# meharkhurana03/cm3d

Hardware: AMD Instinct MI355X
Metric: pseudo-label frames/sec on nuScenes-shaped sweeps (higher is better)
Workload: dtype f32; 1 GPU; c2: 256 frames/GPU x (35000x1 pts, 6 cams, 20 masks 1600x900), masks resident as rle; frames_per_gpu=256, points_per_frame=35000, masks_per_frame=20, lane_points=50000, mask_input=rle, batches_in_flight=4, distinct_batches=4, cloud_materialised=False

## Files before the change

cm3d_amd/_lib.py:

```python
import ctypes as C
import os

_HERE = os.path.dirname(os.path.abspath(__file__))
LIB_PATH = os.environ.get("CM3D_LIB") or os.path.join(_HERE, "libcm3d_hip.so")

ABI_VERSION = 5
CAM_STRIDE = 64
SWEEP_XF_STRIDE = 24
MAX_CAMS = 8
MAX_MASKS_PER_FRAME = 1024
BOX_STRIDE = 10
MEDOID_TILE = 64
STATUS_WORDS = 4
BBOX_STRIDE = 8
MAX_MATCH_BOXES = 1024
MAX_FUSED_SWEEPS = 16
MATCH_BOX_STRIDE = 6
OBB_ROT_STRIDE = 9
WM_BOX_STRIDE = 8
WM_BREAKDOWNS = 16
WM_CUTOFFS = 101
WM_SWEEP_MAX_ALPHAS = 1024
RAW_QUADS = 3

_p, _i32, _i64, _f32 = C.c_void_p, C.c_int32, C.c_int64, C.c_float

SIGNATURES = {
    "cm3d_abi_version": (_i32, []),
    "cm3d_project_workgroups_per_cu": (_i32, [_i32]),
    "cm3d_error_string": (C.c_char_p, [_i32]),
    "cm3d_removed_words": (_i64, [_i32, _i32]),
    "cm3d_batch_begin": (_i32, [_p, _p, _i32, _p, _i64, _p]),
    "cm3d_sweep_prep": (_i32, [_p, _i32, _p, _p, _i32, _i32, _p, _p, _i32, _f32, _p, _i32, _p, _p, _p, _p]),
    "cm3d_rle_workspace_bytes": (_i64, [_i32]),
    "cm3d_rle_to_dense": (_i32, [_p, _p, _i32, _i32, _i32, _i32, _p, _p, _i64, _p]),
    "cm3d_erode_pack": (_i32, [_p, _i32, _i32, _i32, _p, _p, _p]),
    "cm3d_rle_erode_pack": (_i32, [_p, _p, _i32, _i32, _i32, _i32, _p, _p, _p, _i64, _p]),
    "cm3d_rle_erode_pack_begin": (_i32, [_p, _p, _i32, _i32, _i32, _i32, _p, _p, _p, _i64, _p, _p, _i32, _p, _i64, _p]),
    "cm3d_rle_erode_pack_sized": (_i32, [_p, _p, _i32, _i32, _i32, _i32, _p, _p, _p, _p, _i64, _p]),
    "cm3d_rle_erode_pack_sized_begin": (_i32, [_p, _p, _i32, _i32, _i32, _i32, _p, _p, _p, _p, _i64, _p, _p, _i32, _p, _i64, _p]),
    "cm3d_project_workspace_bytes": (_i64, [_i32, _i32, _i32]),
    "cm3d_project_hit_rows": (_i32, [_p, _i64, _i32, _i32, _i32, _p, _p]),
    "cm3d_project_culling": (_i32, [_p, _i64, _i32, _i32, _i32, _p, _p]),
    "cm3d_project_hits": (_i32, [_p, _p, _i32, _i32, _i32, _p, _i32, _p, _p, _p, _p, _i32, _i32, _i32, _f32, _i32,
                                 _p, _p, _p, _p, _i64, _p, _p, _p]),
    "cm3d_sweep_project_hits": (_i32, [_p, _i32, _p, _p, _i32, _i32, _p, _p, _f32, _p, _i32, _p, _p, _i32, _i32, _i32, _p, _i32, _p, _p,
                                       _p, _p, _i32, _i32, _i32, _f32, _i32, _p, _p, _p, _p, _i64, _p, _p, _p]),
    "cm3d_compact_hits": (_i32, [_p, _i32, _i32, _i32, _i32, _p, _i32, _p, _p, _p, _i32, _p, _p, _p, _p, _p, _p, _p, _p, _i32, _p, _p, _p,
                                 _i64, _p]),
    "cm3d_tile_work_bytes": (_i64, [_i32, _i32]),
    "cm3d_selftest_sqrt": (_i32, [C.c_uint32, C.c_uint32, _p, _p, _p]),
    "cm3d_selftest_div": (_i32, [C.c_uint64, C.c_uint64, _p, _p]),
    "cm3d_selftest_mfma": (_i32, [C.c_uint64, _i32, _p, _p]),
    "cm3d_medoid_workspace_bytes": (_i64, [_i32, _i32]),
    "cm3d_medoid": (_i32, [_p, _p, _p, _i32, _p, _p, _p, _i32, _p, _p, _p, _p, _p, _i64, _p]),
    "cm3d_medoid2": (_i32, [_p, _p, _p, _i32, _p, _p, _p, _i32, _p, _p, _p, _p, _p, _i64, _i32, _p, _p]),
    "cm3d_lane_grid_bytes": (_i64, [_i32, _i32]),
    "cm3d_lane_grid_build": (_i32, [_p, _p, _i32, _i32, _p, _i64, _p]),
    "cm3d_lane_nn_workspace_bytes": (_i64, [_i32]),
    "cm3d_lane_nn": (_i32, [_p, _p, _p, _i32, _p, _p, _p, _i32, _i32, _p, _p, _p, _p, _i64, _p]),
    "cm3d_circle_nms": (_i32, [_p, _p, _p, _p, _p, _i32, _p, _i32, _p, _p]),
    "cm3d_box_nms": (_i32, [_p, _p, _p, _i32, _i32, _p, _p, _p, _p, _p, _p, _p, _p, _p, _p, _p, _i32, _p, _p, _p, _p, _p]),
    "cm3d_centroid_transform": (_i32, [_p, _p, _p, _i32, _p, _p, _p]),
    "cm3d_bev_match_workspace_bytes": (_i64, [_i64]),
    "cm3d_bev_match": (_i32, [_p, _p, _i32, _p, _p, _i32, _p, _i32, _i64, C.c_double, _p, _p, _p, _p, _p, _i64, _p]),
    "cm3d_obb_workspace_bytes": (_i64, [_i32, _i32]),
    "cm3d_obb": (_i32, [_p, _p, _i32, _i32, _p, _p, _p, _p, _p, _i64, _p]),
    "cm3d_selftest_obb_yaw": (_i32, [_p, _i32, _p, _p]),
    "cm3d_waymo_metrics_workspace_bytes": (_i64, [_i64]),
    "cm3d_waymo_metrics": (_i32, [_p, _p, _p, _p, _p, _p, _p, _p, _p, _p, _i32, _i64, _i32, _p, _p, _p, _p, _i64, _p]),
    "cm3d_waymo_metrics_sweep_workspace_bytes": (_i64, [_i64]),
    "cm3d_waymo_metrics_sweep": (_i32, [_p, _p, _p, _p, _p, _p, _p, _p, _p, _p, _p, _p, _p, _i32, _i64, _p, _i32, _p, _p, _p, _p, _i64, _p]),
    "cm3d_lift_pass": (_i32, [_p, _p]),
    "cm3d_pipe_exec_streams_for": (_i32, [_i32, _i32]),
    "cm3d_pipe_create": (_p, [_i32, _i32, _p]),
    "cm3d_pipe_destroy": (None, [_p]),
    "cm3d_pipe_exec_streams": (_i32, [_p]),
    "cm3d_pipe_submit": (_i32, [_p, _i32, _p]),
    "cm3d_pipe_submit_timed": (_i32, [_p, _i32, _p, _p, _p]),
    "cm3d_pipe_acquire": (_i32, [_p, _i32]),
    "cm3d_pipe_release": (_i32, [_p, _i32]),
    "cm3d_pipe_wait": (_i32, [_p, _i32]),
    "cm3d_pipe_pin": (_i32, [_p]),
    "cm3d_pipe_last_stream": (_i32, [_p, _i32]),
}


class LiftPassDesc(C.Structure):
    _fields_ = (
        [("size", _i64)]
        + [(n, _p) for n in ("rle_counts", "rle_off", "packed", "bbox", "rle_ws")] + [("rle_ws_bytes", _i64)]
        + [(n, _p) for n in ("status", "hit_count", "removed_bits")] + [("removed_words", _i64)]
        + [(n, _p) for n in ("raw", "intensity", "sweep_row_off", "sweep_xf", "frame_sweep_off", "points", "pt_off", "cams", "mask_off",
                             "mask_cam", "hit_words", "pg_ws")] + [("pg_ws_bytes", _i64)]
        + [(n, _p) for n in ("hit_off", "tile_off", "hit_idx", "hit_xyz", "tile_work", "medoid_pos", "centroid", "colsum", "ws")]
        + [("ws_bytes", _i64), ("md_feedback", _p)]
        + [(n, _p) for n in ("centroid_g", "mask_frame", "lane", "lane_off", "frame_lane", "grid", "lane_idx", "lane_dist", "class_id", "score",
                             "prior_wlh", "is_vehicle", "nms_group", "nms_thr", "ego_xyz", "box", "flags")]
        + [(n, _i32) for n in ("n_masks", "total_runs", "W", "H", "raw_stride", "n_sweeps", "max_sweeps_per_frame", "pt_cap", "n_frames",
                               "max_pts_per_frame", "n_cams", "planes", "idx_cap", "n_tables", "n_lane_points", "n_classes", "md_hint")]
        + [("halfw", _f32), ("min_dist", _f32)])


class Cm3dError(RuntimeError):
    pass


_lib = None


def lib():
    global _lib
    if _lib is None:
        if not os.path.exists(LIB_PATH):
            raise Cm3dError(
                f"{LIB_PATH} is missing: build it with `python -c 'import __graft_entry__ as g; g.build()'` "
                "(hipcc --offload-arch=gfx950).  There is no CPU fallback for the lifting path.")
        handle = C.CDLL(LIB_PATH)
        for name, (res, args) in SIGNATURES.items():
            fn = getattr(handle, name)
            fn.restype = res
            fn.argtypes = args
        if handle.cm3d_abi_version() != ABI_VERSION:
            raise Cm3dError("libcm3d_hip.so ABI version mismatch")
        _lib = handle
    return _lib


def check(code, what):
    if code != 0:
        msg = lib().cm3d_error_string(code).decode()
        raise Cm3dError(f"{what}: {msg} ({code})")
```

cm3d_amd/csrc/boxes.hip:

```cpp
#include "common.h"

#define LG_MAX_CELLS 32768
#define LG_CELL0 4.0f
#define LG_MAX_RINGS 64
#define LG_BIG_CELL 12
#define LG_BUILD_THREADS 1024

struct LaneGrid { float x0, y0, h, inv_h; int gw, gh, cell_base; float margin; };
struct LanePt { float x, y; int idx, pad; };

static __device__ __forceinline__ int lg_cell_coord(float v, float v0, float inv_h, int n)
{
    int c = (int)floorf((v - v0) * inv_h);
    return c < 0 ? 0 : (c >= n ? n - 1 : c);
}

__global__ __launch_bounds__(LG_BUILD_THREADS) void k_lane_grid_build(const float *__restrict__ lane,
                                                                      const int32_t *__restrict__ lane_off,
                                                                      LaneGrid *__restrict__ grids, int32_t *__restrict__ cell_start,
                                                                      LanePt *__restrict__ sorted)
{
    extern __shared__ __align__(16) int s_cell[];
    __shared__ float s_red[4][16];
    __shared__ int s_part[16];
// ... 137 lines not shown
                const int sg = s0 + lane;
                int row, c0, c1;
                if (r_lo == 0) { row = qj - 2 + sg; c0 = qi - 2; c1 = qi + 2; }
                else if (sg < w) { row = qj - r_hi + sg; c0 = qi - r_hi; c1 = qi + r_hi; }
                else if (sg < 2 * w) { row = qj + r_lo + (sg - w); c0 = qi - r_hi; c1 = qi + r_hi; }
                else {
                    const int m = sg - 2 * w;
                    row = qj - r_lo + 1 + (m >> 1);
                    if (m & 1) { c0 = qi + r_lo; c1 = qi + r_hi; } else { c0 = qi - r_hi; c1 = qi - r_lo; }
                }
                c0 = max(c0, 0); c1 = min(c1, g.gw - 1);
                const bool seg_ok = sg < nseg && row >= 0 && row < g.gh && c0 <= c1;
                const int rowc = min(max(row, 0), g.gh - 1), c0c = min(c0, g.gw - 1), c1c = max(c1, 0);
                int a = cs[rowc * g.gw + c0c], b = cs[rowc * g.gw + c1c + 1];
                if (!seg_ok) { a = 0; b = 0; }
                visit(a, b);
            }
            r_done = r_hi;
            const double wb = cm3d_wave_reduce_t(sbest, [](double a, double b) { return fmin(a, b); });
            if (wb < (double)r_done * (double)g.h - (double)g.margin) { resolved = true; break; }
            if (qi - r_done <= 0 && qi + r_done >= g.gw - 1 && qj - r_done <= 0 && qj + r_done >= g.gh - 1) { resolved = true; break; }
        }
    }
    if (!resolved) {
        const int32_t *cs = cell_start + g.cell_base;
        const int a = cs[0], b = cs[g.gw * g.gh];
        for (int q0 = a; q0 < b; q0 += 8 * 64) {
            LanePt p[8];
#pragma unroll
            for (int v = 0; v < 8; ++v) {
                const int q = q0 + v * 64 + lane;
                p[v] = q < b ? sorted[q] : LanePt{0.f, 0.f, 0, 0};
            }
#pragma unroll
            for (int v = 0; v < 8; ++v) {
                if (q0 + v * 64 + lane >= b) continue;
                const double dx = cx - (double)p[v].x, dy = cy - (double)p[v].y;
                lg_consider(dx * dx + dy * dy, p[v].idx, d2cut, sbest, jbest);
            }
        }
    }
    {
        const Cm3dDistIdx best = cm3d_wave_argmin(sbest, jbest);
        sbest = best.s; jbest = best.j;
    }
    if (lane == 0) {
        if (jbest == 0x7FFFFFFF) jbest = 0;
        lane_idx[k] = jbest;
        lane_dist[k] = sbest;
    }
}

static inline size_t lg_align(size_t v) { return (v + 255) & ~(size_t)255; }

struct LgLayout { LaneGrid *grids; int32_t *cell_start; LanePt *sorted; };
static inline LgLayout lg_layout(void *grid, int n_tables, int n_lane_points)
{
    char *w = (char *)grid;
    LgLayout l;
    l.grids = (LaneGrid *)w;          w += lg_align(sizeof(LaneGrid) * (size_t)n_tables);
    l.cell_start = (int32_t *)w;      w += lg_align(sizeof(int32_t) * (size_t)n_tables * (LG_MAX_CELLS + 1));
    l.sorted = (LanePt *)w;
    (void)n_lane_points;
    return l;
}

extern "C" int64_t cm3d_lane_grid_bytes(int32_t n_tables, int32_t n_lane_points)
{
    if (n_tables <= 0 || n_lane_points <= 0) return 0;
    return (int64_t)(lg_align(sizeof(LaneGrid) * (size_t)n_tables) + lg_align(sizeof(int32_t) * (size_t)n_tables * (LG_MAX_CELLS + 1)) +
                     lg_align(sizeof(LanePt) * (size_t)n_lane_points));
}

extern "C" int cm3d_lane_grid_build(const float *lane, const int32_t *lane_off, int32_t n_tables, int32_t n_lane_points, void *grid,
                                    int64_t grid_bytes, cm3d_stream_t stream)
{
    if (!lane || !lane_off || !grid || n_tables <= 0 || n_lane_points <= 0) return CM3D_ERR_ARG;
    if (grid_bytes < cm3d_lane_grid_bytes(n_tables, n_lane_points)) return CM3D_ERR_WORKSPACE;
    const LgLayout l = lg_layout(grid, n_tables, n_lane_points);
    static bool attr_set = false;
    const size_t lds = sizeof(int) * (size_t)(LG_MAX_CELLS + 1);
    if (!attr_set) {
        if (hipFuncSetAttribute((const void *)k_lane_grid_build, hipFuncAttributeMaxDynamicSharedMemorySize, (int)lds) != hipSuccess)
            return CM3D_ERR_LAUNCH;
        attr_set = true;
    }
    hipLaunchKernelGGL(k_lane_grid_build, dim3(n_tables), dim3(LG_BUILD_THREADS), lds, (hipStream_t)stream, lane, lane_off, l.grids,
                       l.cell_start, l.sorted);
    CM3D_CHECK_LAUNCH();
    return CM3D_OK;
}

extern "C" int64_t cm3d_lane_nn_workspace_bytes(int32_t n_masks)
{
    if (n_masks <= 0) return 0;
    return 256;
}

extern "C" int cm3d_lane_nn(const float *centroid, const int32_t *medoid_pos, const int32_t *mask_frame, int32_t n_masks,
                            const float *lane, const int32_t *lane_off, const int32_t *frame_lane, int32_t n_tables,
                            int32_t n_lane_points, const void *grid, int32_t *lane_idx, double *lane_dist, void *workspace,
                            int64_t workspace_bytes, cm3d_stream_t stream)
{
    if (!centroid || !medoid_pos || !mask_frame || !lane || !lane_off || !frame_lane || !grid || !lane_idx || !lane_dist || !workspace)
        return CM3D_ERR_ARG;
    if (n_masks <= 0 || n_tables <= 0 || n_lane_points <= 0) return CM3D_ERR_ARG;
    if (workspace_bytes < cm3d_lane_nn_workspace_bytes(n_masks)) return CM3D_ERR_WORKSPACE;
    const LgLayout l = lg_layout(const_cast<void *>(grid), n_tables, n_lane_points);
    hipLaunchKernelGGL(k_lane_nn_grid, dim3((n_masks + 3) / 4), dim3(256), 0, (hipStream_t)stream, centroid, medoid_pos, mask_frame,
                       n_masks, lane_off, frame_lane, l.grids, l.cell_start, l.sorted, LG_MAX_RINGS, lane_idx, lane_dist);
    CM3D_CHECK_LAUNCH();
    return CM3D_OK;
}

#define BN_MAX CM3D_MAX_MASKS_PER_FRAME

static __device__ __forceinline__ void nms_phase(int nm, int lane_id, const double *__restrict__ nms_thr, const double *s_x,
                                                 const double *s_y, const double *s_s, const int *s_lab, int *s_order,
                                                 const unsigned char *s_valid, unsigned char *s_sup, unsigned char *s_keep)
{
    __syncthreads();
    int nv = 0;
    for (int k = 0; k < nm; ++k) nv += s_valid[k];
    for (int k = lane_id; k < nm; k += 64) {
        if (!s_valid[k]) continue;
        int rank = 0;
        const double sk = s_s[k];
        for (int j = 0; j < nm; ++j) {
            if (!s_valid[j]) continue;
            const double sj = s_s[j];
            rank += (sj > sk || (sj == sk && j > k)) ? 1 : 0;
        }
        s_order[rank] = k;
    }
    __syncthreads();
    for (int r = 0; r < nv; ++r) {
        const int i = s_order[r];
        if (!s_sup[i]) {
            if (lane_id == 0) s_keep[i] = 1;
            const double xi = s_x[i], yi = s_y[i];
            const int li = s_lab[i];
            for (int r2 = r + 1 + lane_id; r2 < nv; r2 += 64) {
                const int j = s_order[r2];
                if (s_sup[j]) continue;
                const double dx = xi - s_x[j], dy = yi - s_y[j];
                const double dist = dx * dx + dy * dy;
                if (dist <= nms_thr[s_lab[j]] && s_lab[j] == li) s_sup[j] = 1;
            }
        }
        __syncthreads();
    }
}

__global__ __launch_bounds__(64) void k_box_nms(const float *__restrict__ centroid, const int32_t *__restrict__ medoid_pos,
                                                const int32_t *__restrict__ mask_off, const int32_t *__restrict__ class_id,
                                                const double *__restrict__ score, const float *__restrict__ lane,
                                                const int32_t *__restrict__ lane_off, const int32_t *__restrict__ frame_lane,
                                                const int32_t *__restrict__ lane_idx, const double *__restrict__ lane_dist,
                                                const double *__restrict__ prior_wlh, const int32_t *__restrict__ is_vehicle,
                                                const int32_t *__restrict__ nms_group, const double *__restrict__ nms_thr,
                                                int n_classes, const double *__restrict__ ego_xyz,
                                                const float *__restrict__ pose_inv, double *__restrict__ box,
                                                int32_t *__restrict__ flags)
{
    __shared__ double s_x[BN_MAX], s_y[BN_MAX], s_s[BN_MAX];
    __shared__ int s_lab[BN_MAX], s_order[BN_MAX];
    __shared__ unsigned char s_valid[BN_MAX], s_sup[BN_MAX], s_keep[BN_MAX];
    const int f = blockIdx.x;
    const int m0 = mask_off[f];
    const int nm = min(mask_off[f + 1] - m0, BN_MAX);
    const int lane_id = threadIdx.x;
    const bool waymo = pose_inv != nullptr;
    const double ex0 = waymo ? 0.0 : ego_xyz[3 * f], ey0 = waymo ? 0.0 : ego_xyz[3 * f + 1];
    double Pi[12];
    if (waymo)
        for (int q = 0; q < 12; ++q) Pi[q] = (double)pose_inv[(size_t)f * 16 + q];
    const int ltab = lane_off[frame_lane[f]];

    for (int k = lane_id; k < nm; k += 64) {
        const int m = m0 + k;
        const int mp = medoid_pos[m], li = lane_idx[m];
        int cls = class_id[m];
        const float c_x = centroid[3 * m], c_y = centroid[3 * m + 1], c_z = centroid[3 * m + 2];
        const double ld_m = lane_dist[m], score_m = score[m];
        const bool valid = mp >= 0;
        if (cls < 0 || cls >= n_classes) cls = 0;
        const float yaw_m = lane[(size_t)(valid ? max(ltab + li, 0) : 0) * 3 + 2];
        const int veh = is_vehicle[cls], grp_c = nms_group[cls];
        const double prior_l = prior_wlh[3 * cls + 0], prior_w = prior_wlh[3 * cls + 1];
        double tx = 0.0, ty = 0.0, tz = 0.0, qw = 1.0, qz = 0.0, yaw_out = 0.0, ld = 0.0;
        if (valid) {
            double cx = (double)c_x, cy = (double)c_y, cz = (double)c_z;
            if (waymo) {
                const double gx = cx, gy = cy, gz = cz;
                cx = Pi[0] * gx + Pi[1] * gy + Pi[2] * gz + Pi[3];
                cy = Pi[4] * gx + Pi[5] * gy + Pi[6] * gz + Pi[7];
                cz = Pi[8] * gx + Pi[9] * gy + Pi[10] * gz + Pi[11];
            }
            const float yaw = yaw_m;
            yaw_out = (double)yaw; ld = ld_m;
            tx = cx; ty = cy; tz = cz;
            if (veh) {
                const double cs = (double)cosf(yaw), sn = (double)sinf(yaw);
                if (cs < -cs) { const double t = 1.0 - cs - cs + 1.0; const double fct = 0.5 / sqrt(t); qw = (sn + sn) * fct; qz = t * fct; }
                else          { const double t = 1.0 + cs + cs + 1.0; const double fct = 0.5 / sqrt(t); qw = t * fct; qz = (sn + sn) * fct; }
                const double PI = 3.14159265358979323846;
                double phi = 2.0 * atan2(qw, qz);
                if (phi > PI) phi -= 2.0 * PI;
                if (phi <= -PI) phi += 2.0 * PI;
                double theta = -phi;
                if (theta != theta) theta = 0.5 * PI;
                const double ex = cx - ex0, ey = cy - ey0;
                double alpha = atan(fabs(ey) / fabs(ex));
                if (ex < 0) { if (ey < 0) alpha = -PI + alpha; else alpha = PI - alpha; }
                else        { if (ey < 0) alpha = -alpha; }
                const double l = prior_l, w = prior_w;
                const double o1 = fabs(w / (2.0 * sin(theta - alpha)));
                const double o2 = fabs(l / (2.0 * cos(theta - alpha)));
                double off = o1 < o2 ? o1 : o2;
                if (o1 != o1 || o2 != o2) off = NAN;
                tx = cx + off * cos(alpha);
                ty = cy + off * sin(alpha);
                if (waymo) {
                    qw = atan2(Pi[4] * cs + Pi[5] * sn, Pi[0] * cs + Pi[1] * sn);
                    qz = 0.0;
                }
            } else if (waymo) {
                qw = 0.0; qz = 0.0;
            }
        }
        double *b = box + (size_t)m * CM3D_BOX_STRIDE;
        b[0] = tx; b[1] = ty; b[2] = tz; b[3] = qw; b[4] = qz; b[5] = yaw_out; b[6] = ld; b[7] = score_m; b[8] = (double)cls;
        s_x[k] = tx; s_y[k] = ty; s_s[k] = score_m; s_lab[k] = grp_c;
        s_valid[k] = valid; s_sup[k] = 0; s_keep[k] = 0;
    }
    nms_phase(nm, lane_id, nms_thr, s_x, s_y, s_s, s_lab, s_order, s_valid, s_sup, s_keep);
    for (int k = lane_id; k < nm; k += 64) {
        const int fl = (s_valid[k] ? 1 : 0) | (s_keep[k] ? 2 : 0);
        flags[m0 + k] = fl;
        box[(size_t)(m0 + k) * CM3D_BOX_STRIDE + 9] = (double)fl;
    }
}

__global__ void k_centroid_transform(const float *__restrict__ cin, const int32_t *__restrict__ medoid_pos,
                                     const int32_t *__restrict__ mask_frame, int n_masks, const float *__restrict__ pose_rt,
                                     float *__restrict__ cout)
{
    const int m = blockIdx.x * blockDim.x + threadIdx.x;
    if (m >= n_masks) return;
    float x = cin[3 * m], y = cin[3 * m + 1], z = cin[3 * m + 2];
    if (medoid_pos[m] >= 0) {
        const float *p = pose_rt + (size_t)mask_frame[m] * 12;
        float ax, ay, az;
        cm3d_rot3(p, x, y, z, ax, ay, az);
        x = ax + p[9]; y = ay + p[10]; z = az + p[11];
    }
    cout[3 * m] = x; cout[3 * m + 1] = y; cout[3 * m + 2] = z;
}

extern "C" int cm3d_centroid_transform(const float *centroid_in, const int32_t *medoid_pos, const int32_t *mask_frame,
                                       int32_t n_masks, const float *pose_rt, float *centroid_out, cm3d_stream_t stream)
{
    if (!centroid_in || !medoid_pos || !mask_frame || !pose_rt || !centroid_out || n_masks <= 0) return CM3D_ERR_ARG;
    hipLaunchKernelGGL(k_centroid_transform, dim3((n_masks + 255) / 256), dim3(256), 0, (hipStream_t)stream, centroid_in, medoid_pos,
                       mask_frame, n_masks, pose_rt, centroid_out);
    CM3D_CHECK_LAUNCH();
    return CM3D_OK;
}

extern "C" int cm3d_box_nms(const float *centroid, const int32_t *medoid_pos, const int32_t *mask_off, int32_t n_frames,
                            int32_t n_masks, const int32_t *class_id, const double *score, const float *lane,
                            const int32_t *lane_off, const int32_t *frame_lane, const int32_t *lane_idx,
                            const double *lane_dist, const double *prior_wlh, const int32_t *is_vehicle,
                            const int32_t *nms_group, const double *nms_thr, int32_t n_classes, const double *ego_xyz,
                            const float *pose_inv, double *box, int32_t *flags, cm3d_stream_t stream)
{
    if (!centroid || !medoid_pos || !mask_off || !class_id || !score || !lane || !lane_off || !frame_lane || !lane_idx ||
        !lane_dist || !prior_wlh || !is_vehicle || !nms_group || !nms_thr || (!ego_xyz && !pose_inv) || !box || !flags)
        return CM3D_ERR_ARG;
    if (n_frames <= 0 || n_masks <= 0 || n_classes <= 0) return CM3D_ERR_ARG;
    hipStream_t st = (hipStream_t)stream;
    hipLaunchKernelGGL(k_box_nms, dim3(n_frames), dim3(64), 0, st, centroid, medoid_pos, mask_off, class_id, score, lane,
                       lane_off, frame_lane, lane_idx, lane_dist, prior_wlh, is_vehicle, nms_group, nms_thr, n_classes, ego_xyz, pose_inv, box, flags);
    CM3D_CHECK_LAUNCH();
    return CM3D_OK;
}


__global__ __launch_bounds__(64) void k_circle_nms(const double *__restrict__ x, const double *__restrict__ y,
                                                   const double *__restrict__ score, const int32_t *__restrict__ label,
                                                   const int32_t *__restrict__ frame_off, const double *__restrict__ nms_thr,
                                                   int n_classes, int32_t *__restrict__ keep)
{
    __shared__ double s_x[BN_MAX], s_y[BN_MAX], s_s[BN_MAX];
    __shared__ int s_lab[BN_MAX], s_order[BN_MAX];
    __shared__ unsigned char s_valid[BN_MAX], s_sup[BN_MAX], s_keep[BN_MAX];
    const int f = blockIdx.x;
    const int m0 = frame_off[f];
    const int nm = min(frame_off[f + 1] - m0, BN_MAX);
    const int lane_id = threadIdx.x;
    for (int k = lane_id; k < nm; k += 64) {
        int cls = label[m0 + k];
        if (cls < 0 || cls >= n_classes) cls = 0;
        s_x[k] = x[m0 + k]; s_y[k] = y[m0 + k]; s_s[k] = score[m0 + k]; s_lab[k] = cls;
        s_valid[k] = 1; s_sup[k] = 0; s_keep[k] = 0;
    }
    nms_phase(nm, lane_id, nms_thr, s_x, s_y, s_s, s_lab, s_order, s_valid, s_sup, s_keep);
    for (int k = lane_id; k < nm; k += 64) keep[m0 + k] = s_keep[k];
}

extern "C" int cm3d_circle_nms(const double *x, const double *y, const double *score, const int32_t *label,
                               const int32_t *frame_off, int32_t n_frames, const double *nms_thr, int32_t n_classes,
                               int32_t *keep, cm3d_stream_t stream)
{
    if (!x || !y || !score || !label || !frame_off || !nms_thr || !keep) return CM3D_ERR_ARG;
    if (n_frames <= 0 || n_classes <= 0) return CM3D_ERR_ARG;
    hipLaunchKernelGGL(k_circle_nms, dim3(n_frames), dim3(64), 0, (hipStream_t)stream, x, y, score, label, frame_off, nms_thr,
                       n_classes, keep);
    CM3D_CHECK_LAUNCH();
    return CM3D_OK;
}

extern "C" int cm3d_abi_version(void) { return CM3D_ABI_VERSION; }

extern "C" const char *cm3d_error_string(int code)
{
    switch (code) {
    case CM3D_OK: return "ok";
    case CM3D_ERR_ARG: return "invalid argument (null pointer, non-positive size or unsupported shape)";
    case CM3D_ERR_LAUNCH: return "kernel launch failed";
    case CM3D_ERR_WORKSPACE: return "workspace too small";
    default: return "unknown error";
    }
}
```

cm3d_amd/csrc/pipeline.cpp:

```cpp
#include <hip/hip_runtime_api.h>

#include <cstdlib>
#include <new>

#include "../../include/cm3d_hip.h"
#include "pipe_sched.h"

static int lift_pass(const cm3d_lift_pass_desc *d, void *ev_start, void *ev_stop, cm3d_stream_t st)
{
    if (!d || d->size != (int64_t)sizeof(cm3d_lift_pass_desc)) return CM3D_ERR_ARG;
    int rc = cm3d_rle_erode_pack_begin(d->rle_counts, d->rle_off, d->n_masks, d->total_runs, d->W, d->H, d->packed, d->bbox, d->rle_ws,
                                       d->rle_ws_bytes, d->status, d->hit_count, d->n_masks, d->removed_bits, d->removed_words, st);
    if (rc != CM3D_OK) return rc;
    rc = cm3d_sweep_project_hits(d->raw, d->raw_stride, d->intensity, d->sweep_row_off, d->n_sweeps, d->max_sweeps_per_frame, d->sweep_xf,
                                 d->frame_sweep_off, d->halfw, d->points, d->pt_cap, d->pt_off, d->removed_bits, d->n_frames,
                                 d->max_pts_per_frame, d->pt_cap, d->cams, d->n_cams, d->mask_off, d->mask_cam, d->bbox, d->packed, d->n_masks,
                                 d->W, d->H, d->min_dist, d->planes, d->hit_words, d->hit_count, d->status, d->pg_ws, d->pg_ws_bytes,
                                 ev_start, ev_stop, st);
    if (rc != CM3D_OK) return rc;
    const bool from_raw = d->points == nullptr;
    rc = cm3d_compact_hits(d->hit_words, d->planes, d->n_frames, d->max_pts_per_frame, d->pt_cap, d->mask_off, d->n_masks, d->hit_count,
                           d->removed_bits, from_raw ? d->raw : nullptr, d->raw_stride, from_raw ? d->intensity : nullptr,
                           from_raw ? d->sweep_xf : nullptr, d->points, d->hit_off, d->tile_off, d->hit_idx, nullptr, d->hit_xyz, d->idx_cap,
                           d->tile_work, d->status, d->pg_ws, d->pg_ws_bytes, st);
    if (rc != CM3D_OK) return rc;
    int32_t md_flags = 0;
    if (d->md_hint && d->md_feedback && *(const volatile int32_t *)d->md_feedback == 0) md_flags = 1;
    rc = cm3d_medoid2(d->hit_xyz, nullptr, nullptr, d->n_masks, d->hit_off, d->tile_off, nullptr, d->idx_cap, d->tile_work, d->medoid_pos,
                      d->centroid, d->colsum, d->ws, d->ws_bytes, md_flags, d->md_feedback, st);
    if (rc != CM3D_OK) return rc;
    rc = cm3d_lane_nn(d->centroid_g, d->medoid_pos, d->mask_frame, d->n_masks, d->lane, d->lane_off, d->frame_lane, d->n_tables,
                      d->n_lane_points, d->grid, d->lane_idx, d->lane_dist, d->ws, d->ws_bytes, st);
    if (rc != CM3D_OK) return rc;
    return cm3d_box_nms(d->centroid_g, d->medoid_pos, d->mask_off, d->n_frames, d->n_masks, d->class_id, d->score, d->lane, d->lane_off,
                        d->frame_lane, d->lane_idx, d->lane_dist, d->prior_wlh, d->is_vehicle, d->nms_group, d->nms_thr, d->n_classes,
                        d->ego_xyz, nullptr, d->box, d->flags, st);
}

extern "C" int cm3d_lift_pass(const cm3d_lift_pass_desc *d, cm3d_stream_t st) { return lift_pass(d, nullptr, nullptr, st); }

extern "C" int cm3d_pipe_exec_streams_for(int32_t depth, int32_t hw_queues)
{
    if (hw_queues <= 0) hw_queues = cm3d::pipe_hw_queues(std::getenv("GPU_MAX_HW_QUEUES"));
    return cm3d::pipe_exec_streams(depth, hw_queues);
}

namespace {

struct Pipe {
    cm3d::PipeSched sched;
    hipStream_t streams[cm3d::kPipeMaxDepth];
    hipEvent_t done[cm3d::kPipeMaxDepth];
    bool recorded[cm3d::kPipeMaxDepth];
    Pipe(int depth, int n_exec) : sched(depth, n_exec) {}
};

int pipe_take(Pipe *p, int32_t slot)
{
    if (!p || slot < 0 || slot >= p->sched.depth) return CM3D_ERR_ARG;
    const cm3d::PipeTicket t = p->sched.next(slot);
    if (t.wait && p->recorded[slot] && hipEventQuery(p->done[slot]) != hipSuccess) {
        (void)hipGetLastError();
        if (hipStreamWaitEvent(p->streams[t.stream], p->done[slot], 0) != hipSuccess) return CM3D_ERR_LAUNCH;
    }
    return t.stream;
}

int pipe_mark(Pipe *p, int32_t slot)
{
    const int s = p->sched.last[slot];
    if (s < 0) return CM3D_ERR_ARG;
    if (hipEventRecord(p->done[slot], p->streams[s]) != hipSuccess) return CM3D_ERR_LAUNCH;
    p->recorded[slot] = true;
    return CM3D_OK;
}

}

extern "C" void *cm3d_pipe_create(int32_t depth, int32_t exec_streams, const cm3d_stream_t *streams)
{
    if (depth < 1 || depth > cm3d::kPipeMaxDepth || !streams) return nullptr;
    const int n_exec = exec_streams > 0 ? (exec_streams < depth ? exec_streams : depth) : cm3d_pipe_exec_streams_for(depth, 0);
    Pipe *p = new (std::nothrow) Pipe(depth, n_exec);
    if (!p) return nullptr;
    for (int i = 0; i < cm3d::kPipeMaxDepth; ++i) {
        p->streams[i] = nullptr;
        p->done[i] = nullptr;
        p->recorded[i] = false;
    }
    for (int i = 0; i < depth; ++i) {
        p->streams[i] = (hipStream_t)streams[i];
        if (hipEventCreateWithFlags(&p->done[i], hipEventDisableTiming) != hipSuccess) {
            cm3d_pipe_destroy(p);
            return nullptr;
        }
    }
    return p;
}

extern "C" void cm3d_pipe_destroy(void *pipe)
{
    Pipe *p = (Pipe *)pipe;
    if (!p) return;
    for (int i = 0; i < p->sched.depth; ++i)
        if (p->done[i]) (void)hipEventDestroy(p->done[i]);
    delete p;
}

extern "C" int cm3d_pipe_exec_streams(const void *pipe)
{
    return pipe ? ((const Pipe *)pipe)->sched.n_exec : CM3D_ERR_ARG;
}

extern "C" int cm3d_pipe_submit(void *pipe, int32_t slot, const cm3d_lift_pass_desc *desc)
{
    return cm3d_pipe_submit_timed(pipe, slot, desc, nullptr, nullptr);
}

extern "C" int cm3d_pipe_submit_timed(void *pipe, int32_t slot, const cm3d_lift_pass_desc *desc, void *ev_start, void *ev_stop)
{
    Pipe *p = (Pipe *)pipe;
    if (!desc) return CM3D_ERR_ARG;
    const int s = pipe_take(p, slot);
    if (s < 0) return s;
    const int rc = lift_pass(desc, ev_start, ev_stop, (cm3d_stream_t)p->streams[s]);
    const int rm = pipe_mark(p, slot);
    if (rc != CM3D_OK) return rc;
    return rm != CM3D_OK ? rm : s;
}

extern "C" int cm3d_pipe_acquire(void *pipe, int32_t slot) { return pipe_take((Pipe *)pipe, slot); }

extern "C" int cm3d_pipe_release(void *pipe, int32_t slot)
{
    Pipe *p = (Pipe *)pipe;
    if (!p || slot < 0 || slot >= p->sched.depth) return CM3D_ERR_ARG;
    return pipe_mark(p, slot);
}

extern "C" int cm3d_pipe_wait(void *pipe, int32_t slot)
{
    Pipe *p = (Pipe *)pipe;
    if (!p || slot < 0 || slot >= p->sched.depth) return CM3D_ERR_ARG;
    if (!p->recorded[slot]) return CM3D_OK;
    return hipEventSynchronize(p->done[slot]) == hipSuccess ? CM3D_OK : CM3D_ERR_LAUNCH;
}

extern "C" int cm3d_pipe_pin(void *pipe)
{
    if (!pipe) return CM3D_ERR_ARG;
    ((Pipe *)pipe)->sched.pin();
    return CM3D_OK;
}

extern "C" int cm3d_pipe_last_stream(const void *pipe, int32_t slot)
{
    const Pipe *p = (const Pipe *)pipe;
    if (!p || slot < 0 || slot >= p->sched.depth) return CM3D_ERR_ARG;
    return p->sched.last[slot];
}
```

include/cm3d_hip.h:

```cpp
#ifndef CM3D_HIP_H
#define CM3D_HIP_H

#include <stdint.h>

#ifdef __cplusplus
extern "C" {
#endif

#define CM3D_ABI_VERSION 5

#define CM3D_OK 0
#define CM3D_ERR_ARG (-1)
#define CM3D_ERR_LAUNCH (-2)
#define CM3D_ERR_WORKSPACE (-3)

#define CM3D_CAM_STRIDE 64
#define CM3D_SWEEP_XF_STRIDE 24
#define CM3D_RAW_QUADS 3
#define CM3D_MAX_CAMS 8
#define CM3D_MAX_MASKS_PER_FRAME 1024
#define CM3D_BBOX_STRIDE 8
#define CM3D_BOX_STRIDE 10
#define CM3D_MEDOID_TILE 64
#define CM3D_MAX_MATCH_BOXES 1024
#define CM3D_MATCH_BOX_STRIDE 6
#define CM3D_OBB_ROT_STRIDE 9
#define CM3D_WM_BOX_STRIDE 8
#define CM3D_WM_BREAKDOWNS 16
#define CM3D_WM_CUTOFFS 101
#define CM3D_WM_SWEEP_MAX_ALPHAS 1024

#define CM3D_STATUS_WORDS 4

typedef void *cm3d_stream_t;

int cm3d_abi_version(void);
const char *cm3d_error_string(int code);

int64_t cm3d_removed_words(int32_t n_rows, int32_t n_frames);
int cm3d_batch_begin(int32_t *status, int32_t *hit_count, int32_t n_masks, uint32_t *removed_bits, int64_t removed_words,
                     cm3d_stream_t stream);

int cm3d_sweep_prep(const float *raw, int32_t raw_stride, const float *intensity, const int32_t *sweep_row_off, int32_t n_sweeps,
                    int32_t max_rows_per_sweep, const float *sweep_xf, const int32_t *frame_sweep_off,
                    int32_t n_frames, float halfw, float *points, int32_t pt_cap, int32_t *pt_off,
                    uint32_t *removed_bits, int32_t *status, cm3d_stream_t stream);

int64_t cm3d_rle_workspace_bytes(int32_t total_runs);
int cm3d_rle_to_dense(const uint32_t *rle_counts, const int32_t *rle_off, int32_t n_masks, int32_t total_runs,
                      int32_t W, int32_t H, uint8_t *dense, void *workspace, int64_t workspace_bytes,
                      cm3d_stream_t stream);

int cm3d_erode_pack(const uint8_t *dense, int32_t n_masks, int32_t W, int32_t H, uint32_t *packed,
                    int32_t *bbox, cm3d_stream_t stream);

int cm3d_rle_erode_pack(const uint32_t *rle_counts, const int32_t *rle_off, int32_t n_masks, int32_t total_runs,
                        int32_t W, int32_t H, uint32_t *packed, int32_t *bbox, void *workspace,
                        int64_t workspace_bytes, cm3d_stream_t stream);

int cm3d_rle_erode_pack_begin(const uint32_t *rle_counts, const int32_t *rle_off, int32_t n_masks, int32_t total_runs,
                              int32_t W, int32_t H, uint32_t *packed, int32_t *bbox, void *workspace, int64_t workspace_bytes,
                              int32_t *status, int32_t *hit_count, int32_t n_count_masks, uint32_t *removed_bits, int64_t removed_words,
                              cm3d_stream_t stream);

int cm3d_rle_erode_pack_sized(const uint32_t *rle_counts, const int32_t *rle_off, int32_t n_masks, int32_t total_runs,
                              int32_t W, int32_t H, const int32_t *mask_wh, uint32_t *packed, int32_t *bbox, void *workspace,
                              int64_t workspace_bytes, cm3d_stream_t stream);

int cm3d_rle_erode_pack_sized_begin(const uint32_t *rle_counts, const int32_t *rle_off, int32_t n_masks, int32_t total_runs,
                                    int32_t W, int32_t H, const int32_t *mask_wh, uint32_t *packed, int32_t *bbox, void *workspace,
                                    int64_t workspace_bytes, int32_t *status, int32_t *hit_count, int32_t n_count_masks,
                                    uint32_t *removed_bits, int64_t removed_words, cm3d_stream_t stream);

int64_t cm3d_project_workspace_bytes(int32_t n_frames, int32_t max_pts_per_frame, int32_t planes);
int cm3d_project_hit_rows(const void *workspace, int64_t workspace_bytes, int32_t n_frames, int32_t max_pts_per_frame,
                          int32_t planes, int64_t *rows_out, cm3d_stream_t stream);
int cm3d_project_culling(const void *workspace, int64_t workspace_bytes, int32_t n_frames, int32_t max_pts_per_frame,
                         int32_t planes, int32_t *out, cm3d_stream_t stream);
int cm3d_project_hits(const float *points, const int32_t *pt_off, int32_t n_frames, int32_t max_pts_per_frame,
                      int32_t n_points_total, const float *cams, int32_t n_cams, const int32_t *mask_off,
                      const int32_t *mask_cam, const int32_t *bbox, const uint32_t *packed, int32_t n_masks,
                      int32_t W, int32_t H, float min_dist, int32_t planes, uint32_t *hit_words,
                      int32_t *hit_count, int32_t *status, void *workspace, int64_t workspace_bytes,
                      void *ev_start, void *ev_stop, cm3d_stream_t stream);

#define CM3D_MAX_FUSED_SWEEPS 16
int cm3d_project_workgroups_per_cu(int32_t n);

int cm3d_sweep_project_hits(const float *raw, int32_t raw_stride, const float *intensity, const int32_t *sweep_row_off, int32_t n_sweeps,
                            int32_t max_sweeps_per_frame, const float *sweep_xf, const int32_t *frame_sweep_off,
                            float halfw, float *points, int32_t pt_cap, int32_t *pt_off, uint32_t *removed_bits,
                            int32_t n_frames, int32_t max_pts_per_frame, int32_t n_points_total,
                            const float *cams, int32_t n_cams, const int32_t *mask_off, const int32_t *mask_cam,
                            const int32_t *bbox, const uint32_t *packed, int32_t n_masks, int32_t W, int32_t H,
                            float min_dist, int32_t planes, uint32_t *hit_words, int32_t *hit_count, int32_t *status,
                            void *workspace, int64_t workspace_bytes, void *ev_start, void *ev_stop, cm3d_stream_t stream);

int cm3d_compact_hits(const uint32_t *hit_words, int32_t planes, int32_t n_frames, int32_t max_pts_per_frame,
                      int32_t n_points_total, const int32_t *mask_off, int32_t n_masks, const int32_t *hit_count,
                      const uint32_t *removed_bits, const float *raw, int32_t raw_stride, const float *intensity, const float *sweep_xf,
                      const float *points, int32_t *hit_off, int32_t *tile_off, int32_t *hit_idx, int32_t *hit_row,
                      float *hit_xyz, int32_t idx_cap, int32_t *tile_work, int32_t *status, void *workspace,
                      int64_t workspace_bytes, cm3d_stream_t stream);
int64_t cm3d_tile_work_bytes(int32_t n_masks, int32_t idx_cap);

int64_t cm3d_medoid_workspace_bytes(int32_t n_masks, int32_t idx_cap);
int cm3d_medoid(const float *points, const int32_t *pt_off, const int32_t *mask_frame, int32_t n_masks,
                const int32_t *hit_off, const int32_t *tile_off, const int32_t *hit_row, int32_t idx_cap,
                const int32_t *tile_work, int32_t *medoid_pos, float *centroid, float *colsum_opt, void *workspace,
                int64_t workspace_bytes, cm3d_stream_t stream);
int cm3d_medoid2(const float *points, const int32_t *pt_off, const int32_t *mask_frame, int32_t n_masks,
                 const int32_t *hit_off, const int32_t *tile_off, const int32_t *hit_row, int32_t idx_cap,
                 const int32_t *tile_work, int32_t *medoid_pos, float *centroid, float *colsum_opt, void *workspace,
                 int64_t workspace_bytes, int32_t flags, int32_t *feedback, cm3d_stream_t stream);

int cm3d_selftest_div(uint64_t seed, uint64_t count, uint64_t *n_bad, cm3d_stream_t stream);

int cm3d_selftest_mfma(uint64_t seed, int32_t tiles_per_wave, uint64_t *n_bad, cm3d_stream_t stream);

int cm3d_selftest_sqrt(uint32_t first_bits, uint32_t last_bits, uint64_t *n_bad, uint32_t *first_bad, cm3d_stream_t stream);

int64_t cm3d_lane_grid_bytes(int32_t n_tables, int32_t n_lane_points);
int cm3d_lane_grid_build(const float *lane, const int32_t *lane_off, int32_t n_tables, int32_t n_lane_points, void *grid,
                         int64_t grid_bytes, cm3d_stream_t stream);
int64_t cm3d_lane_nn_workspace_bytes(int32_t n_masks);
int cm3d_lane_nn(const float *centroid, const int32_t *medoid_pos, const int32_t *mask_frame, int32_t n_masks,
                 const float *lane, const int32_t *lane_off, const int32_t *frame_lane, int32_t n_tables,
                 int32_t n_lane_points, const void *grid, int32_t *lane_idx, double *lane_dist, void *workspace,
                 int64_t workspace_bytes, cm3d_stream_t stream);

int cm3d_box_nms(const float *centroid, const int32_t *medoid_pos, const int32_t *mask_off, int32_t n_frames,
                 int32_t n_masks, const int32_t *class_id, const double *score, const float *lane,
                 const int32_t *lane_off, const int32_t *frame_lane, const int32_t *lane_idx,
                 const double *lane_dist, const double *prior_wlh, const int32_t *is_vehicle,
                 const int32_t *nms_group, const double *nms_thr, int32_t n_classes, const double *ego_xyz,
                 const float *pose_inv, double *box, int32_t *flags, cm3d_stream_t stream);

int cm3d_centroid_transform(const float *centroid_in, const int32_t *medoid_pos, const int32_t *mask_frame,
                            int32_t n_masks, const float *pose_rt, float *centroid_out, cm3d_stream_t stream);

int cm3d_circle_nms(const double *x, const double *y, const double *score, const int32_t *label,
                    const int32_t *frame_off, int32_t n_frames, const double *nms_thr, int32_t n_classes,
                    int32_t *keep, cm3d_stream_t stream);

int64_t cm3d_bev_match_workspace_bytes(int64_t total_pairs);
int cm3d_bev_match(const double *pred, const int32_t *pred_off, int32_t n_pred, const double *gt,
                   const int32_t *gt_off, int32_t n_gt, const int64_t *pair_off, int32_t n_frames,
                   int64_t total_pairs, double iou_thr, int32_t *pred_match, int32_t *gt_match, double *match_iou,
                   int32_t *status, void *workspace, int64_t workspace_bytes, cm3d_stream_t stream);

int64_t cm3d_obb_workspace_bytes(int32_t n_masks, int32_t idx_cap);
int cm3d_obb(const float *hit_xyz, const int32_t *hit_off, int32_t n_masks, int32_t idx_cap, double *yaw, int32_t *obb_status,
             double *rot_opt, uint8_t *vertex_opt, void *workspace, int64_t workspace_bytes, cm3d_stream_t stream);

int cm3d_selftest_obb_yaw(const double *R, int32_t n, double *yaw, cm3d_stream_t stream);

int64_t cm3d_waymo_metrics_workspace_bytes(int64_t total_pairs);
int cm3d_waymo_metrics(const double *pred_box, const float *pred_heading, const float *pred_score, const int32_t *pred_off,
                       const double *gt_box, const float *gt_heading, const int32_t *gt_level, const int32_t *gt_off,
                       const int32_t *group_bd, const int64_t *pair_off, int32_t n_groups, int64_t total_pairs,
                       int32_t per_cutoff, int64_t *counts, int64_t *heading_sum, int32_t *status, void *workspace,
                       int64_t workspace_bytes, cm3d_stream_t stream);

int64_t cm3d_waymo_metrics_sweep_workspace_bytes(int64_t total_pairs);
int cm3d_waymo_metrics_sweep(const double *cand_box, const float *cand_heading, const int32_t *cand_kind, const double *cand_p,
                             const double *cand_s, const int32_t *cand_off, const double *gt_box, const float *gt_heading,
                             const int32_t *gt_level, const int32_t *gt_off, const int32_t *group_bd, const int64_t *pair_off,
                             const int32_t *group_static, int32_t n_groups, int64_t total_pairs, const double *alphas,
                             int32_t n_alphas, int64_t *counts, int64_t *heading_sum, int32_t *status, void *workspace,
                             int64_t workspace_bytes, cm3d_stream_t stream);

typedef struct cm3d_lift_pass_desc {
    int64_t size;
    const uint32_t *rle_counts; const int32_t *rle_off; uint32_t *packed; int32_t *bbox; void *rle_ws; int64_t rle_ws_bytes;
    int32_t *status; int32_t *hit_count; uint32_t *removed_bits; int64_t removed_words;
    const float *raw; const float *intensity; const int32_t *sweep_row_off; const float *sweep_xf; const int32_t *frame_sweep_off;
    float *points; int32_t *pt_off; const float *cams; const int32_t *mask_off; const int32_t *mask_cam; uint32_t *hit_words;
    void *pg_ws; int64_t pg_ws_bytes;
    int32_t *hit_off; int32_t *tile_off; int32_t *hit_idx; float *hit_xyz; int32_t *tile_work; int32_t *medoid_pos; float *centroid;
    float *colsum; void *ws; int64_t ws_bytes;
    int32_t *md_feedback;
    const float *centroid_g; const int32_t *mask_frame; const float *lane; const int32_t *lane_off; const int32_t *frame_lane;
    const void *grid; int32_t *lane_idx; double *lane_dist; const int32_t *class_id; const double *score; const double *prior_wlh;
    const int32_t *is_vehicle; const int32_t *nms_group; const double *nms_thr; const double *ego_xyz; double *box; int32_t *flags;
    int32_t n_masks, total_runs, W, H, raw_stride, n_sweeps, max_sweeps_per_frame, pt_cap, n_frames, max_pts_per_frame, n_cams, planes,
            idx_cap, n_tables, n_lane_points, n_classes;
    int32_t md_hint;
    float halfw, min_dist;
} cm3d_lift_pass_desc;

int cm3d_lift_pass(const cm3d_lift_pass_desc *desc, cm3d_stream_t stream);

int cm3d_pipe_exec_streams_for(int32_t depth, int32_t hw_queues);

void *cm3d_pipe_create(int32_t depth, int32_t exec_streams, const cm3d_stream_t *streams);
void cm3d_pipe_destroy(void *pipe);
int cm3d_pipe_exec_streams(const void *pipe);
int cm3d_pipe_submit(void *pipe, int32_t slot, const cm3d_lift_pass_desc *desc);
int cm3d_pipe_submit_timed(void *pipe, int32_t slot, const cm3d_lift_pass_desc *desc, void *ev_start, void *ev_stop);
int cm3d_pipe_acquire(void *pipe, int32_t slot);
int cm3d_pipe_release(void *pipe, int32_t slot);
int cm3d_pipe_wait(void *pipe, int32_t slot);
int cm3d_pipe_pin(void *pipe);
int cm3d_pipe_last_stream(const void *pipe, int32_t slot);

#ifdef __cplusplus
}
#endif
#endif
```

Baseline: 2.331 million frames/s.

## Bound box-NMS shared memory and run small frames' NMS in registers with wave ballots

The box NMS kernel now sizes its shared arrays dynamically from a per-frame mask cap taken from the lift-pass plane count, instead of a fixed BN_MAX static allocation. Frames with at most 64 masks keep their state in registers and do ranking and suppression with readlane and ballot, with no LDS traffic or barriers. The kernel is also templated on Waymo versus nuScenes to drop runtime branches and the unused pose registers. Masks beyond the cap get a zeroed, not-kept box, so output depends on the planes-derived cap being a true upper bound.

```diff
diff --git a/cm3d_amd/_lib.py b/cm3d_amd/_lib.py
--- a/cm3d_amd/_lib.py
+++ b/cm3d_amd/_lib.py
@@ -61,6 +61,7 @@
     "cm3d_lane_nn": (_i32, [_p, _p, _p, _i32, _p, _p, _p, _i32, _i32, _p, _p, _p, _p, _i64, _p]),
     "cm3d_circle_nms": (_i32, [_p, _p, _p, _p, _p, _i32, _p, _i32, _p, _p]),
     "cm3d_box_nms": (_i32, [_p, _p, _p, _i32, _i32, _p, _p, _p, _p, _p, _p, _p, _p, _p, _p, _p, _i32, _p, _p, _p, _p, _p]),
+    "cm3d_box_nms_bounded": (_i32, [_p, _p, _p, _i32, _i32, _p, _p, _p, _p, _p, _p, _p, _p, _p, _p, _p, _i32, _p, _p, _i32, _p, _p, _p]),
     "cm3d_centroid_transform": (_i32, [_p, _p, _p, _i32, _p, _p, _p]),
     "cm3d_bev_match_workspace_bytes": (_i64, [_i64]),
     "cm3d_bev_match": (_i32, [_p, _p, _i32, _p, _p, _i32, _p, _i32, _i64, C.c_double, _p, _p, _p, _p, _p, _i64, _p]),
diff --git a/cm3d_amd/csrc/boxes.hip b/cm3d_amd/csrc/boxes.hip
--- a/cm3d_amd/csrc/boxes.hip
+++ b/cm3d_amd/csrc/boxes.hip
@@ -313,6 +313,14 @@
     }
 }
 
+static __device__ __forceinline__ double bn_readlane(double v, int src)
+{
+    return __hiloint2double(__builtin_amdgcn_readlane(__double2hiint(v), src), __builtin_amdgcn_readlane(__double2loint(v), src));
+}
+
+static inline size_t bn_lds_bytes(int cap) { return cap <= 64 ? 0 : (size_t)((cap + 7) & ~7) * (3 * sizeof(double) + 2 * sizeof(int) + 3); }
+
+template <bool WAYMO>
 __global__ __launch_bounds__(64) void k_box_nms(const float *__restrict__ centroid, const int32_t *__restrict__ medoid_pos,
                                                 const int32_t *__restrict__ mask_off, const int32_t *__restrict__ class_id,
                                                 const double *__restrict__ score, const float *__restrict__ lane,
@@ -321,22 +329,28 @@
                                                 const double *__restrict__ prior_wlh, const int32_t *__restrict__ is_vehicle,
                                                 const int32_t *__restrict__ nms_group, const double *__restrict__ nms_thr,
                                                 int n_classes, const double *__restrict__ ego_xyz,
-                                                const float *__restrict__ pose_inv, double *__restrict__ box,
+                                                const float *__restrict__ pose_inv, int cap, double *__restrict__ box,
                                                 int32_t *__restrict__ flags)
 {
-    __shared__ double s_x[BN_MAX], s_y[BN_MAX], s_s[BN_MAX];
-    __shared__ int s_lab[BN_MAX], s_order[BN_MAX];
-    __shared__ unsigned char s_valid[BN_MAX], s_sup[BN_MAX], s_keep[BN_MAX];
+    extern __shared__ __align__(8) double s_bn[];
+    const int cap8 = (cap + 7) & ~7;
+    double *const s_x = s_bn, *const s_y = s_x + cap8, *const s_s = s_y + cap8;
+    int *const s_lab = reinterpret_cast<int *>(s_s + cap8), *const s_order = s_lab + cap8;
+    unsigned char *const s_valid = reinterpret_cast<unsigned char *>(s_order + cap8), *const s_sup = s_valid + cap8, *const s_keep = s_sup + cap8;
     const int f = blockIdx.x;
     const int m0 = mask_off[f];
-    const int nm = min(mask_off[f + 1] - m0, BN_MAX);
+    const int nm_all = min(mask_off[f + 1] - m0, BN_MAX);
+    const int nm = min(nm_all, cap);
     const int lane_id = threadIdx.x;
-    const bool waymo = pose_inv != nullptr;
-    const double ex0 = waymo ? 0.0 : ego_xyz[3 * f], ey0 = waymo ? 0.0 : ego_xyz[3 * f + 1];
-    double Pi[12];
-    if (waymo)
+    const bool in_regs = nm <= 64;
+    const double ex0 = WAYMO ? 0.0 : ego_xyz[3 * f], ey0 = WAYMO ? 0.0 : ego_xyz[3 * f + 1];
+    double Pi[WAYMO ? 12 : 1];
+    if (WAYMO)
         for (int q = 0; q < 12; ++q) Pi[q] = (double)pose_inv[(size_t)f * 16 + q];
     const int ltab = lane_off[frame_lane[f]];
+    double r_x = 0.0, r_y = 0.0, r_s = 0.0, r_thr = 0.0;
+    int r_lab = 0;
+    bool r_valid = false;
 
     for (int k = lane_id; k < nm; k += 64) {
         const int m = m0 + k;
@@ -349,10 +363,11 @@
         const float yaw_m = lane[(size_t)(valid ? max(ltab + li, 0) : 0) * 3 + 2];
         const int veh = is_vehicle[cls], grp_c = nms_group[cls];
         const double prior_l = prior_wlh[3 * cls + 0], prior_w = prior_wlh[3 * cls + 1];
+        if (in_regs && valid) r_thr = nms_thr[grp_c];
         double tx = 0.0, ty = 0.0, tz = 0.0, qw = 1.0, qz = 0.0, yaw_out = 0.0, ld = 0.0;
         if (valid) {
             double cx = (double)c_x, cy = (double)c_y, cz = (double)c_z;
-            if (waymo) {
+            if (WAYMO) {
                 const double gx = cx, gy = cy, gz = cz;
                 cx = Pi[0] * gx + Pi[1] * gy + Pi[2] * gz + Pi[3];
                 cy = Pi[4] * gx + Pi[5] * gy + Pi[6] * gz + Pi[7];
@@ -382,24 +397,64 @@
                 if (o1 != o1 || o2 != o2) off = NAN;
                 tx = cx + off * cos(alpha);
                 ty = cy + off * sin(alpha);
-                if (waymo) {
+                if (WAYMO) {
                     qw = atan2(Pi[4] * cs + Pi[5] * sn, Pi[0] * cs + Pi[1] * sn);
                     qz = 0.0;
                 }
-            } else if (waymo) {
+            } else if (WAYMO) {
                 qw = 0.0; qz = 0.0;
             }
         }
         double *b = box + (size_t)m * CM3D_BOX_STRIDE;
         b[0] = tx; b[1] = ty; b[2] = tz; b[3] = qw; b[4] = qz; b[5] = yaw_out; b[6] = ld; b[7] = score_m; b[8] = (double)cls;
-        s_x[k] = tx; s_y[k] = ty; s_s[k] = score_m; s_lab[k] = grp_c;
-        s_valid[k] = valid; s_sup[k] = 0; s_keep[k] = 0;
-    }
-    nms_phase(nm, lane_id, nms_thr, s_x, s_y, s_s, s_lab, s_order, s_valid, s_sup, s_keep);
-    for (int k = lane_id; k < nm; k += 64) {
-        const int fl = (s_valid[k] ? 1 : 0) | (s_keep[k] ? 2 : 0);
-        flags[m0 + k] = fl;
-        box[(size_t)(m0 + k) * CM3D_BOX_STRIDE + 9] = (double)fl;
+        if (in_regs) {
+            r_x = tx; r_y = ty; r_s = score_m; r_lab = grp_c; r_valid = valid;
+        } else {
+            s_x[k] = tx; s_y[k] = ty; s_s[k] = score_m; s_lab[k] = grp_c;
+            s_valid[k] = valid; s_sup[k] = 0; s_keep[k] = 0;
+        }
+    }
+    if (in_regs) {
+        const uint64_t vmask = __ballot(r_valid);
+        int rank = 0;
+        for (int j = 0; j < nm; ++j) {
+            const double sj = bn_readlane(r_s, j);
+            if ((vmask >> j) & 1) rank += (sj > r_s || (sj == r_s && j > lane_id)) ? 1 : 0;
+        }
+        const int nv = (int)__popcll(vmask);
+        uint64_t sup = 0, keep = 0;
+        for (int r = 0; r < nv; ++r) {
+            const uint64_t sel = __ballot(r_valid && rank == r);
+            if (!sel) continue;
+            const int i = (int)__builtin_ctzll(sel);
+            if ((sup >> i) & 1) continue;
+            keep |= 1ull << i;
+            const double xi = bn_readlane(r_x, i), yi = bn_readlane(r_y, i);
+            const int li = __builtin_amdgcn_readlane(r_lab, i);
+            const double dx = xi - r_x, dy = yi - r_y;
+            const double dist = dx * dx + dy * dy;
+            sup |= __ballot(r_valid && rank > r && dist <= r_thr && r_lab == li);
+        }
+        if (lane_id < nm) {
+            const int fl = (r_valid ? 1 : 0) | ((keep >> lane_id) & 1 ? 2 : 0);
+            flags[m0 + lane_id] = fl;
+            box[(size_t)(m0 + lane_id) * CM3D_BOX_STRIDE + 9] = (double)fl;
+        }
+    } else {
+        nms_phase(nm, lane_id, nms_thr, s_x, s_y, s_s, s_lab, s_order, s_valid, s_sup, s_keep);
+        for (int k = lane_id; k < nm; k += 64) {
+            const int fl = (s_valid[k] ? 1 : 0) | (s_keep[k] ? 2 : 0);
+            flags[m0 + k] = fl;
+            box[(size_t)(m0 + k) * CM3D_BOX_STRIDE + 9] = (double)fl;
+        }
+    }
+    for (int k = nm + lane_id; k < nm_all; k += 64) {
+        const int m = m0 + k;
+        int cls = class_id[m];
+        if (cls < 0 || cls >= n_classes) cls = 0;
+        double *b = box + (size_t)m * CM3D_BOX_STRIDE;
+        b[0] = 0.0; b[1] = 0.0; b[2] = 0.0; b[3] = 1.0; b[4] = 0.0; b[5] = 0.0; b[6] = 0.0; b[7] = score[m]; b[8] = (double)cls; b[9] = 0.0;
+        flags[m] = 0;
     }
 }
 
@@ -429,6 +484,30 @@
     return CM3D_OK;
 }
 
+extern "C" int cm3d_box_nms_bounded(const float *centroid, const int32_t *medoid_pos, const int32_t *mask_off, int32_t n_frames,
+                                    int32_t n_masks, const int32_t *class_id, const double *score, const float *lane,
+                                    const int32_t *lane_off, const int32_t *frame_lane, const int32_t *lane_idx,
+                                    const double *lane_dist, const double *prior_wlh, const int32_t *is_vehicle,
+                                    const int32_t *nms_group, const double *nms_thr, int32_t n_classes, const double *ego_xyz,
+                                    const float *pose_inv, int32_t max_masks_per_frame, double *box, int32_t *flags, cm3d_stream_t stream)
+{
+    if (!centroid || !medoid_pos || !mask_off || !class_id || !score || !lane || !lane_off || !frame_lane || !lane_idx ||
+        !lane_dist || !prior_wlh || !is_vehicle || !nms_group || !nms_thr || (!ego_xyz && !pose_inv) || !box || !flags)
+        return CM3D_ERR_ARG;
+    if (n_frames <= 0 || n_masks <= 0 || n_classes <= 0 || max_masks_per_frame <= 0) return CM3D_ERR_ARG;
+    hipStream_t st = (hipStream_t)stream;
+    const int cap = max_masks_per_frame < BN_MAX ? max_masks_per_frame : BN_MAX;
+    const size_t lds = bn_lds_bytes(cap);
+    if (pose_inv)
+        hipLaunchKernelGGL(k_box_nms<true>, dim3(n_frames), dim3(64), lds, st, centroid, medoid_pos, mask_off, class_id, score, lane,
+                           lane_off, frame_lane, lane_idx, lane_dist, prior_wlh, is_vehicle, nms_group, nms_thr, n_classes, ego_xyz, pose_inv, cap, box, flags);
+    else
+        hipLaunchKernelGGL(k_box_nms<false>, dim3(n_frames), dim3(64), lds, st, centroid, medoid_pos, mask_off, class_id, score, lane,
+                           lane_off, frame_lane, lane_idx, lane_dist, prior_wlh, is_vehicle, nms_group, nms_thr, n_classes, ego_xyz, pose_inv, cap, box, flags);
+    CM3D_CHECK_LAUNCH();
+    return CM3D_OK;
+}
+
 extern "C" int cm3d_box_nms(const float *centroid, const int32_t *medoid_pos, const int32_t *mask_off, int32_t n_frames,
                             int32_t n_masks, const int32_t *class_id, const double *score, const float *lane,
                             const int32_t *lane_off, const int32_t *frame_lane, const int32_t *lane_idx,
@@ -436,15 +515,9 @@
                             const int32_t *nms_group, const double *nms_thr, int32_t n_classes, const double *ego_xyz,
                             const float *pose_inv, double *box, int32_t *flags, cm3d_stream_t stream)
 {
-    if (!centroid || !medoid_pos || !mask_off || !class_id || !score || !lane || !lane_off || !frame_lane || !lane_idx ||
-        !lane_dist || !prior_wlh || !is_vehicle || !nms_group || !nms_thr || (!ego_xyz && !pose_inv) || !box || !flags)
-        return CM3D_ERR_ARG;
-    if (n_frames <= 0 || n_masks <= 0 || n_classes <= 0) return CM3D_ERR_ARG;
-    hipStream_t st = (hipStream_t)stream;
-    hipLaunchKernelGGL(k_box_nms, dim3(n_frames), dim3(64), 0, st, centroid, medoid_pos, mask_off, class_id, score, lane,
-                       lane_off, frame_lane, lane_idx, lane_dist, prior_wlh, is_vehicle, nms_group, nms_thr, n_classes, ego_xyz, pose_inv, box, flags);
-    CM3D_CHECK_LAUNCH();
-    return CM3D_OK;
+    return cm3d_box_nms_bounded(centroid, medoid_pos, mask_off, n_frames, n_masks, class_id, score, lane, lane_off, frame_lane, lane_idx,
+                                lane_dist, prior_wlh, is_vehicle, nms_group, nms_thr, n_classes, ego_xyz, pose_inv, CM3D_MAX_MASKS_PER_FRAME,
+                                box, flags, stream);
 }
 
 
diff --git a/cm3d_amd/csrc/pipeline.cpp b/cm3d_amd/csrc/pipeline.cpp
--- a/cm3d_amd/csrc/pipeline.cpp
+++ b/cm3d_amd/csrc/pipeline.cpp
@@ -32,9 +32,10 @@
     rc = cm3d_lane_nn(d->centroid_g, d->medoid_pos, d->mask_frame, d->n_masks, d->lane, d->lane_off, d->frame_lane, d->n_tables,
                       d->n_lane_points, d->grid, d->lane_idx, d->lane_dist, d->ws, d->ws_bytes, st);
     if (rc != CM3D_OK) return rc;
-    return cm3d_box_nms(d->centroid_g, d->medoid_pos, d->mask_off, d->n_frames, d->n_masks, d->class_id, d->score, d->lane, d->lane_off,
-                        d->frame_lane, d->lane_idx, d->lane_dist, d->prior_wlh, d->is_vehicle, d->nms_group, d->nms_thr, d->n_classes,
-                        d->ego_xyz, nullptr, d->box, d->flags, st);
+    return cm3d_box_nms_bounded(d->centroid_g, d->medoid_pos, d->mask_off, d->n_frames, d->n_masks, d->class_id, d->score, d->lane,
+                                d->lane_off, d->frame_lane, d->lane_idx, d->lane_dist, d->prior_wlh, d->is_vehicle, d->nms_group, d->nms_thr,
+                                d->n_classes, d->ego_xyz, nullptr, d->planes > 0 && d->planes < CM3D_MAX_MASKS_PER_FRAME / 32 ? 32 * d->planes : CM3D_MAX_MASKS_PER_FRAME,
+                                d->box, d->flags, st);
 }
 
 extern "C" int cm3d_lift_pass(const cm3d_lift_pass_desc *d, cm3d_stream_t st) { return lift_pass(d, nullptr, nullptr, st); }
diff --git a/include/cm3d_hip.h b/include/cm3d_hip.h
--- a/include/cm3d_hip.h
+++ b/include/cm3d_hip.h
@@ -135,6 +135,12 @@
                  const double *lane_dist, const double *prior_wlh, const int32_t *is_vehicle,
                  const int32_t *nms_group, const double *nms_thr, int32_t n_classes, const double *ego_xyz,
                  const float *pose_inv, double *box, int32_t *flags, cm3d_stream_t stream);
+int cm3d_box_nms_bounded(const float *centroid, const int32_t *medoid_pos, const int32_t *mask_off, int32_t n_frames,
+                         int32_t n_masks, const int32_t *class_id, const double *score, const float *lane,
+                         const int32_t *lane_off, const int32_t *frame_lane, const int32_t *lane_idx,
+                         const double *lane_dist, const double *prior_wlh, const int32_t *is_vehicle,
+                         const int32_t *nms_group, const double *nms_thr, int32_t n_classes, const double *ego_xyz,
+                         const float *pose_inv, int32_t max_masks_per_frame, double *box, int32_t *flags, cm3d_stream_t stream);
 
 int cm3d_centroid_transform(const float *centroid_in, const int32_t *medoid_pos, const int32_t *mask_frame,
                             int32_t n_masks, const float *pose_rt, float *centroid_out, cm3d_stream_t stream);
```

New measurement: 2.367 million frames/s (median of 6 runs). 1.02x the previous value.
